# LukeFrankio/CiviWave-FEM

Hardware: AMD Instinct MI355X
Metric: PCG DOF-iterations/sec per Newmark step (PCG-it/s x DOFs); DOF-updates/s and K_eff HBM GB/s vs roofline reported alongside (higher is better)
Workload: dtype f32 SpMV, fp16-packed block-Jacobi, f64 reductions

## Files before the change

civiwave-fem_amd/csrc/cwf_internal.hpp:

```cpp
#pragma once

#include <hip/hip_runtime.h>

#include <cstdint>
#include <initializer_list>
#include <string>
#include <vector>

#include "../../include/cwf_hip.h"
#include "devmem.hpp"
#include "knobs.hpp"

namespace cwf
{

constexpr int kTileElems = 512;
constexpr int kMaxTileNodes = 512;
uint32_t hex_tile_lanes(uint64_t hexes);
#ifndef CWF_GROUP_SLOTS
#define CWF_GROUP_SLOTS 12
#endif
#ifndef CWF_GROUP_WAVES
#define CWF_GROUP_WAVES 1
#endif
// ... 195 lines not shown
    DevTiles t{};
};

struct Ctl
{
    double rho, alpha, beta, tol, res, rhs_norm, rhs_norm_raw, alpha_last, beta_last, denom, rr, rz;
    unsigned long long iterations;
    int active;
    int converged;
    int error;
    int error_iter;
    double rho2[2];
    double alpha_h[kXLag];
};

enum class PcgSchedule
{
    Parity,
    TwoKernel,
    Fused,
    FusedPeer,
    Resident,
};
struct SchedulePlan
{
    enum State
    {
        Unplanned,
        Local,
        Decided
    } state = Unplanned;
    unsigned grid = 0;
    int fused_knob = -1;
    PcgSchedule launch = PcgSchedule::TwoKernel;
    bool resident = false;
};

struct ResidentPlan
{
    unsigned G = 0, npt = 0, nph = 0;
    unsigned own_stride = 0, halo_stride = 0, npub = 0;
    size_t lds = 0;
    unsigned dims[3] = {0, 0, 0};
    unsigned max_own = 0, max_halo = 0;
    uint64_t halo_total = 0;
    const uint4 *hdr = nullptr, *own = nullptr, *halo = nullptr;
    const float4 *tcoef = nullptr;
    float *pub = nullptr;
    double *sh = nullptr;
    uint32_t tag = 1;
    bool shard = false;
    uint64_t remote_sends = 0;
    uint64_t ghost_total = 0;
};


const char *dashpot_update(const double C[9], double mass, double alpha, double dt, double P[9], double Q[9]);

}

struct cwf_hip_system
{
    cwf_hip_system() = default;
    cwf_hip_system(cwf_hip_system &&) = default;
    ~cwf_hip_system();
    int device = 0;
    hipStream_t stream = nullptr;
    int mode = CWF_MODE_PARITY;
    cwf::DevSys ds{};
    uint64_t reduction_block = 256;
    uint64_t reduction_partials = 1;
    cwf::DeviceArena mem;
    float *x = nullptr, *r = nullptr, *p = nullptr, *z = nullptr, *Ap = nullptr, *rhs = nullptr, *tmp = nullptr;
    float *p2 = nullptr, *p3 = nullptr, *p4 = nullptr;
    float *r2 = nullptr, *ap2 = nullptr;
    double *fsh = nullptr;
    double *g_fsh = nullptr;
    bool cls_global = false;
    bool unusable = false;
    int32_t px_send_k[2] = {-1, -1};
    uint32_t px_ebase = 0;
    cwf::SchedulePlan sched;
    cwf::ResidentPlan res;
    float *inv = nullptr;
    float *inv6 = nullptr;
    bool inv_fast = false;
    double inv_sK = 0.0, inv_sM = 0.0;
    double *part0 = nullptr, *part1 = nullptr, *part2 = nullptr;
    double *fgran = nullptr;
    uint32_t fgran_tag = 0;
    uint64_t part_cap = 0;
    uint32_t *perm = nullptr;
    float *pbuf = nullptr;
    cwf::Ctl *ctl = nullptr;
    cwf::Ctl *ctl_host = nullptr;
    double *scal = nullptr;
    cwf::DevicePtr<double> hist;
    uint64_t hist_cap = 0;
    uint64_t hist_count = 0;
    std::vector<uint32_t> lat_plane;
    uint64_t last_iters = 0, prev_iters = 0;
    std::string err, ctx;
    float *mo_blk = nullptr;
    uint32_t mo_cols = 0;
    double *mo_f64 = nullptr;
    float *mo_mass = nullptr;
// ... 228 lines not shown
```

civiwave-fem_amd/csrc/knobs.hpp:

```cpp
#pragma once

#include <cstdlib>
#include <cstring>

namespace cwf
{
struct Knob
{
    const char *name;
    const char *doc;
};

inline constexpr Knob kKnobs[] = {
    {"CWF_RENUMBER", "0: keep the caller's node order (no Morton / owner-tile renumbering)"},
    {"CWF_GEO", "0: the 48-B gradient records instead of recomputing geometry from tile-node coordinates"},
    {"CWF_GROUPS", "0: per-tet tiles (k_keff_tiles_pipe) instead of the fan groups"},
    {"CWF_GROUP_NT", "128: 128-lane fan-group tiles (default 256; tests/test_gpu_parity.py)"},
    {"CWF_TILE_ORDER", "morton|rcb: per-tet / hex8 tile order"},
    {"CWF_TILE_PIPE", "0: the one-tile-per-workgroup per-tet kernel (k_keff_tiles)"},
    {"CWF_HEX_NT", "128|256: lanes of the hex8 tiles (tests/test_hex8.py)"},
    {"CWF_LATTICE", "0: no structured-block stencil (lattice.cpp); structured Kuhn (hex8) blocks then run the fan groups (hex tiles)"},
    {"CWF_LAT_ZR", "0|1: the lattice update pass stores z / the K_eff pass forms z from r and the node class "
                   "(default: the latter from 2M nodes)"},
    {"CWF_LAT_L", "n: planes per lattice brick (default: about 1024 bricks of 256 threads, at least 4 planes)"},
    {"CWF_PARITY_TILES", "strip: PARITY node tiles of 256 consecutive nodes also on a single handle (default there: "
                         "compact breadth-first tiles and a separate p.Ap partials pass; shards always use strips)"},
    {"CWF_PARITY_STREAM", "0: the PARITY loop folds alpha / beta in their own kernels (k_pcg_alpha / k_pcg_beta) instead "
                          "of in workgroup 0 of the pass producing the chunk partials (kernels_parity.hip fold_stream)"},
    {"CWF_RESIDENT", "0: a structured block that fits on chip runs the launch-per-iteration schedules instead of the "
                     "resident one-launch solve (resident.hip; also off whenever CWF_FUSED is set)"},
    {"CWF_FUSED", "0: structured blocks run the two-kernel iteration (k_keff_lattice + k_pcg_update_tiles) instead of "
                  "the fused one-launch iteration (lattice_fused.inc); 2: fused also where the grid walks the work items "
                  "persistently (default: fused only where one round of workgroups covers them)"},
    {"CWF_PEER_FUSED", "0: a PEER shard's fused iteration exchanges through a k_peer_step launch after each fused launch "
                       "instead of inside the launch (lattice_fused.inc fused_peer_wait / fused_peer_publish)"},
    {"CWF_FUSED_TRACE", "path (ablation build only): per-workgroup phase stamps of one fused launch per solve, appended"},
    {"CWF_RESIDENT_TRACE", "path: per-workgroup phase stamps of one phase (CWF_FUSED_TRACE_IT) of every resident solve, "
                           "appended (tools/resident_trace.py)"},
    {"CWF_RESIDENT_REREAD", "1: every phase of the resident solve takes its first ring vote as failed once, so every ring "
                            "granule is requested and formed twice (tests/test_gpu_resident_handoff.py: same bits)"},
    {"CWF_FUSED_TRACE_IT", "n: the iteration whose launch CWF_FUSED_TRACE records (default 50)"},
    {"CWF_FUSED_MAXWG", "n: cap on the fused launch's grid (default 1024 workgroups; a grid below the work items walks them persistently)"},
    {"CWF_XLAG", "1..4: iterations per lazy x update (tests/test_gpu_parity.py compares 4 with 1)"},
    {"CWF_RCCL_LIB", "path: load this NCCL-API library instead of librccl (tests/transport: the host-staged "
                     "test transport that runs several ranks on one GPU, where RCCL refuses duplicate devices)"},
    {"CWF_TIMED_PCG", "bits: cwf_hip_keff_timed times the PCG-mode tiles kernel dry (tools/ablate.py)"},
    {"CWF_VERBOSE", "1: print the tiling statistics at create"},
};

inline const char *knob(const char *name)
{
    for (const Knob &k : kKnobs)
        if (std::strcmp(k.name, name) == 0)
            return std::getenv(name);
    return nullptr;
}
}
```

civiwave-fem_amd/csrc/lattice_common.hpp:

```cpp
#pragma once

#include <hip/hip_runtime.h>

#include <cstddef>
#include <type_traits>

#include "cwf_internal.hpp"
#include "keff_pick.hpp"
#include "reduce.hpp"

namespace cwf
{
namespace
{
typedef uint32_t u32x3 __attribute__((ext_vector_type(3)));
typedef float f2 __attribute__((ext_vector_type(2)));

__device__ __forceinline__ __amdgpu_buffer_rsrc_t ctl_rsrc(const Ctl *c)
{
    return __builtin_amdgcn_make_buffer_rsrc(const_cast<Ctl *>(c), 0, (int)sizeof(Ctl), 0x00020000);
}
__device__ __forceinline__ double ctl_f64(__amdgpu_buffer_rsrc_t rs, uint32_t off)
{
    const uint32_t lo = __builtin_amdgcn_raw_buffer_load_b32(rs, off, 0, 0),
// ... 28 lines not shown
struct LatHex
{
    static constexpr int nOff = kLatHexOffsets, nPairs = kLatHexPairs, coefPairs = 9 * kLatHexOffsets;
    static constexpr const int (&off)[kLatHexOffsets][3] = kLatHexOff;
    static constexpr int pair[kLatHexPairs][2] = {
#define P8(c) {c, 0}, {c, 1}, {c, 2}, {c, 3}, {c, 4}, {c, 5}, {c, 6}, {c, 7}
        P8(0), P8(1), P8(2), P8(3), P8(4), P8(5), P8(6), P8(7)
#undef P8
    };
    static constexpr const int (&pairOff)[kLatHexPairs] = kLatHexPairOff;
    static constexpr int pairStart[9] = {0, 8, 16, 24, 32, 40, 48, 56, 64};
};
template <bool HEX> using LatE = std::conditional_t<HEX, LatHex, LatKuhn>;
template <class E> constexpr const char *lat_kind() { return std::is_same_v<E, LatHex> ? "LatHex" : "LatKuhn"; }
constexpr uint32_t kLatOob3 = 0x15555555u;
constexpr uint32_t kLatOob1 = 0x3FFFFFFFu;

template <bool AFF>
__device__ __forceinline__ uint32_t lat_plane(const DevTiles &T, const uint32_t *__restrict__ plane, int k)
{
    if constexpr (AFF)
        return (uint32_t)k * T.lpstride;
    else
        return plane[k];
}

__device__ __forceinline__ __amdgpu_buffer_rsrc_t sized_rsrc(const void *base, uint32_t bytes)
{
    return __builtin_amdgcn_make_buffer_rsrc(const_cast<void *>(base), 0, (int)bytes, 0x00020000);
}

__device__ __forceinline__ void lat_z(const float4 A, const float2 B, uint32_t cls, const float r[3], float z[3])
{
    const float iv[9] = {A.x, A.y, A.z, A.y, A.w, B.x, A.z, B.x, B.y};
#pragma unroll
    for (int k = 0; k < 3; ++k)
    {
        const float zk = fmaf(iv[3 * k + 2], r[2], fmaf(iv[3 * k + 1], r[1], iv[3 * k] * r[0]));
        z[k] = (cls >> k) & 1u ? 0.0f : zk;
    }
}

enum
{
    kFR = 0,
    kFRR = 1,
    kFPA = 2,
    kFZA = 3,
    kFAMA = 4,
    kFusedShares = 5,
    kFusedSlot = 8
};

__device__ __forceinline__ bool fused_decide(Ctl *ctl, double *hist, unsigned j, const CtlPre &pre,
                                             const double v[kFusedShares], float *alpha_out, float *beta_out)
{
    const unsigned it = j - 1u;
    const double res = sqrt(v[kFRR]);
    const bool conv = it > 0 && res <= pre.tol;
    const double rho = v[kFR], denom = v[kFPA];
    const bool derr = !conv && fabs(denom) < 1.0e-18;
    const bool rerr = !conv && !derr && fabs(rho) < 1.0e-18;
    const double alpha = (conv || derr || rerr) ? 0.0 : rho / denom;
    const double rho_next = rho - 2.0 * alpha * v[kFZA] + alpha * alpha * v[kFAMA];
    const double beta = (conv || derr || rerr) ? 0.0 : rho_next / rho;
    if (blockIdx.x == 0 && threadIdx.x == 0)
    {
        if (it > 0)
        {
            ctl->res = res;
            ctl->iterations = it;
            hist[it] = res;
        }
        ctl->denom = denom;
        if (conv)
        {
            ctl->converged = 1;
            ctl->active = 0;
        }
        else if (derr)
        {
            ctl->error = CWF_ERR_DENOM_ZERO;
            ctl->error_iter = (int)it;
            ctl->active = 0;
        }
        else if (rerr)
        {
            ctl->error = CWF_ERR_RHO_ZERO;
            ctl->error_iter = (int)it;
            ctl->active = 0;
        }
        else
        {
            ctl->alpha = alpha;
            ctl->alpha_last = alpha;
            ctl->rho2[it & 1u] = rho;
            ctl->beta = beta;
            ctl->beta_last = beta;
        }
    }
    *alpha_out = (float)alpha;
    *beta_out = (float)beta;
    return !(conv || derr || rerr);
}

__device__ __forceinline__ void fused_form(const float4 *czA, const float2 *czB, uint32_t cls, float alpha,
                                           float beta, const float r[3], const float a[3], const float p[3],
                                           float rn[3], float z[3], float pn[3])
{
#pragma unroll
    for (int c = 0; c < 3; ++c)
        rn[c] = (cls >> c) & 1u ? 0.f : fmaf(-alpha, a[c], r[c]);
    lat_z(czA[cls], czB[cls], cls, rn, z);
#pragma unroll
    for (int c = 0; c < 3; ++c)
        pn[c] = fmaf(beta, p[c], z[c]);
}

__device__ __forceinline__ void fused_row_dots(const float4 *czA, const float2 *czB, uint32_t cls, const float u[3],
// ... 21 lines not shown
```

civiwave-fem_amd/csrc/lattice_fused.inc:

```

struct FusedArgs
{
    Ctl *ctl;
    const double *sin;
    unsigned nin;
    unsigned sin_stride, sis;
    double *sout;
    unsigned sstride;
    unsigned j;
    unsigned grid;
    double *hist;
    const float *rin;
    float *rout;
    const float *ain;
    float *aout;
    const float *pin;
    float *pout;
    float *x;
    unsigned px;
    FusedPeerArgs pe;
    uint64_t *trace;
};

constexpr uint64_t kFusedPeerTimeoutTicks = 10ull * 100000000ull;
// ... 54 lines not shown
    __shared__ int last_s;
    asm volatile("s_waitcnt vmcnt(0)" ::: "memory");
    __syncthreads();
    if (threadIdx.x == 0)
        last_s = __hip_atomic_fetch_add(pe.ticket, 1u, __ATOMIC_RELAXED, __HIP_MEMORY_SCOPE_AGENT) + 1u == gridDim.x;
    __syncthreads();
    if (!last_s)
        return;
    __builtin_amdgcn_fence(__ATOMIC_ACQUIRE, "");
    double v[kFusedShares];
    fold_k<NT, kFusedShares>(fa.sout, gridDim.x, fa.sstride, red, v);
    if (threadIdx.x < kFusedSlot)
    {
        double t = 0.0;
#pragma unroll
        for (int q = 0; q < kFusedShares; ++q)
            t = threadIdx.x == (unsigned)q ? v[q] : t;
        for (uint32_t p = 0; p < pe.nranks; ++p)
            __hip_atomic_store(pe.gdst[p] + threadIdx.x, t, __ATOMIC_RELAXED, __HIP_MEMORY_SCOPE_SYSTEM);
    }
    asm volatile("s_waitcnt vmcnt(0)" ::: "memory");
    __syncthreads();
    if (threadIdx.x == 0)
    {
        __builtin_amdgcn_fence(__ATOMIC_RELEASE, "");
        for (uint32_t p = 0; p < pe.nranks; ++p)
            if (p != pe.rank)
                __hip_atomic_store(pe.flag[p], pe.epoch, __ATOMIC_RELAXED, __HIP_MEMORY_SCOPE_SYSTEM);
        __hip_atomic_store(pe.done, pe.epoch, __ATOMIC_RELAXED, __HIP_MEMORY_SCOPE_SYSTEM);
        __hip_atomic_store(pe.ticket, 0u, __ATOMIC_RELAXED, __HIP_MEMORY_SCOPE_AGENT);
    }
}

__device__ __forceinline__ void st3_sys(__amdgpu_buffer_rsrc_t rs, uint32_t byteoff, const float v[3])
{
    const u32x3 w = {__float_as_uint(v[0]), __float_as_uint(v[1]), __float_as_uint(v[2])};
    __builtin_amdgcn_raw_buffer_store_b96(w, rs, byteoff, 0, 17);
}

template <int NT>
__device__ __forceinline__ bool fused_scalars(const FusedArgs &fa, const CtlPre &pre, double *red, float *alpha_out,
                                              float *beta_out)
{
    if (fa.j == 0)
    {
        *alpha_out = 0.f;
        *beta_out = 0.f;
        return pre.active != 0;
    }
    double v[kFusedShares];
    fold_k<NT, kFusedShares>(fa.sin, fa.nin, fa.sin_stride, red, v, fa.sis);
    if (!pre.active)
        return false;
    return fused_decide(fa.ctl, fa.hist, fa.j, pre, v, alpha_out, beta_out);
}

struct FusedFill
{
    float r[2][3], a[2][3], p[2][3];
    uint32_t c[2];
    float x[3], m;
};

struct FusedKeep
{
    float z[3], m;
    uint32_t c;
};

template <class E, bool AFF, bool SHARD>
__device__ __forceinline__ void fused_shell_node(const DevSys &s, const FusedArgs &fa, const float *__restrict__ coef,
                                                 const uint32_t *__restrict__ plane, uint32_t q, float alpha,
                                                 float beta, const float4 *czA, const float2 *czB,
                                                 double d[kFusedShares])
{
    const DevTiles &T = s.t;
    const int nx = (int)T.lnx, ny = (int)T.lny, nz = (int)T.lnz;
    int i, j, k;
    uint32_t rq = q;
    const uint32_t full = (uint32_t)(nx * ny), per = (uint32_t)(2 * nx + 2 * (ny - 2));
    const uint32_t nlo = T.lk0 == 0 ? full : 0u, nmid = (T.lkI1 - T.lkI0) * per;
    if (rq < nlo)
    {
        k = 0;
        i = (int)(rq % (uint32_t)nx);
        j = (int)(rq / (uint32_t)nx);
    }
    else if ((rq -= nlo) < nmid)
    {
        k = (int)(T.lkI0 + rq / per);
        rq %= per;
        if (rq < (uint32_t)nx)
            i = (int)rq, j = 0;
        else if (rq < 2u * nx)
            i = (int)rq - nx, j = ny - 1;
        else if (rq < 2u * nx + (uint32_t)(ny - 2))
            i = 0, j = 1 + (int)rq - 2 * nx;
        else
            i = nx - 1, j = 1 + (int)rq - 2 * nx - (ny - 2);
    }
    else
    {
        rq -= nmid;
        k = nz - 1;
        i = (int)(rq % (uint32_t)nx);
        j = (int)(rq / (uint32_t)nx);
    }
// ... 577 lines not shown
```

civiwave-fem_amd/csrc/resident.cpp:

```cpp
#include <algorithm>
#include <cstdio>
#include <cstring>

#include "abi_internal.hpp"

namespace cwf
{
namespace
{
constexpr unsigned kResThreads = 512, kResOwn = 4 * kResThreads, kResHalo = 3 * kResThreads;
constexpr unsigned kResTypesHost = 12;
constexpr unsigned kResGhostHost = 512;
constexpr uint32_t kNone = 0xFFFFFFFFu;
constexpr uint32_t kResGhost = 0x80000000u;
constexpr unsigned kFusedSharesHost = 5;

void split(unsigned n, unsigned g, unsigned q, unsigned &a, unsigned &b)
{
    a = (unsigned)((uint64_t)n * q / g);
    b = (unsigned)((uint64_t)n * (q + 1) / g);
}
}

bool plan_resident(cwf_hip_system *h, bool shard)
// ... 160 lines not shown
                    for (int o = 1; o < noff; ++o)
                    {
                        const long ii = (long)i + off[o][0], jj = (long)j + off[o][1], kk = (long)k + off[o][2];
                        if (!inside(ii, jj, kk))
                            continue;
                        const uint32_t m = node((unsigned)ii, (unsigned)jj, (unsigned)kk);
                        if (owner[m] == b || seen[m] == b)
                            continue;
                        seen[m] = b;
                        const unsigned slot = (unsigned)((kk - (long)q[4] + 1) * PXY + (jj - (long)q[2] + 1) * PX +
                                                         (ii - (long)q[0] + 1));
                        const uint32_t src = m >= Nown ? kResGhost | (m - Nown) : pubidx[m];
                        halol[b].push_back(uint4{m, slot, src, 0u});
                    }
        std::sort(halol[b].begin(), halol[b].end(), [](const uint4 &a, const uint4 &c) { return a.z < c.z; });
        max_halo = std::max<unsigned>(max_halo, (unsigned)halol[b].size());
        halo_total += halol[b].size();
        const auto g0 = std::find_if(halol[b].begin(), halol[b].end(), [](const uint4 &e) { return (e.z & kResGhost) != 0; });
        const uint64_t ng = (uint64_t)(halol[b].end() - g0);
        if (ng > kResGhostHost)
            return false;
        hdr[b].y = (uint32_t)(g0 - halol[b].begin());
        ghost_total += ng;
    }
    const bool small0 = (max_own + kResThreads - 1) / kResThreads <= 3 && (max_halo + kResThreads - 1) / kResThreads <= 2;
    std::vector<uint8_t> btypes((size_t)G * kResTypesHost, 0);
    for (unsigned b = 0; b < G && !small0; ++b)
    {
        int idx[27];
        std::fill(idx, idx + 27, -1);
        unsigned nt = 0;
        for (const uint4 &e : ownl[b])
            idx[cls[e.x] >> 3] = 0;
        for (unsigned ty = 0; ty < 27; ++ty)
            if (idx[ty] == 0 && ty != 13)
            {
                if (nt == kResTypesHost)
                    return false;
                btypes[(size_t)b * kResTypesHost + nt] = (uint8_t)ty;
                idx[ty] = (int)nt++;
            }
        for (uint4 &e : ownl[b])
        {
            const unsigned ty = cls[e.x] >> 3;
            e.y |= (ty == 13 ? 0u : (uint32_t)idx[ty]) << 24;
        }
    }
    const unsigned npt = (max_own + kResThreads - 1) / kResThreads, nph = (max_halo + kResThreads - 1) / kResThreads;
    if (max_own > kResOwn || max_halo > kResHalo || max_slots > slot_cap(max_own, max_halo) || N - Nown >= kResGhost)
        return false;
    const bool small = npt <= 3 && nph <= 2;
    const unsigned own_stride = (small ? 3u : 4u) * kResThreads, halo_stride = (small ? 2u : 3u) * kResThreads;
    const size_t lds = max_slots * 16;
    if (resident_blocks_per_cu(h->ds, npt, nph, lds, shard) < 1)
        return false;
    std::vector<uint4> own((size_t)G * own_stride, uint4{kNone, 0u, kNone, kNone}),
        halo((size_t)G * halo_stride, uint4{kNone, 0u, kNone, 0u});
    for (unsigned b = 0; b < G; ++b)
    {
        std::copy(ownl[b].begin(), ownl[b].end(), own.begin() + (size_t)b * own_stride);
        std::copy(halol[b].begin(), halol[b].end(), halo.begin() + (size_t)b * halo_stride);
    }
    const int npairs = t.lhex ? kLatHexPairs : kLatPairs;
    std::vector<float> cf((size_t)(noff + npairs) * 9);
    if (hipMemcpy(cf.data(), t.lcoef, cf.size() * sizeof(float), hipMemcpyDeviceToHost) != hipSuccess)
        return false;
    std::vector<float4> tco(27ull * noff * 3, float4{0.f, 0.f, 0.f, 0.f});
    for (unsigned ty = 0; ty < 27; ++ty)
    {
        const unsigned sd[3] = {ty % 3, (ty / 3) % 3, ty / 9};
        unsigned w8 = 0;
        for (unsigned c8 = 0; c8 < 8; ++c8)
        {
            bool in = true;
            for (int ax = 0; ax < 3; ++ax)
                in = in && (((c8 >> ax) & 1u) ? sd[ax] != 0 : sd[ax] != 2);
            w8 |= (in ? 1u : 0u) << c8;
        }
        for (int o = 1; o < noff; ++o)
        {
            double S[9] = {};
            for (int pp = 0; pp < npairs; ++pp)
            {
                const int c = t.lhex ? pp / 8 : kLatPair[pp][0];
                const int po = t.lhex ? kLatHexPairOff[pp] : kLatPairOff[pp];
                if (po != o || !((w8 >> c) & 1u))
                    continue;
                for (int e = 0; e < 9; ++e)
                    S[e] += (double)cf[(size_t)9 * noff + 9 * pp + e];
            }
            float4 *q = &tco[(size_t)3 * (ty * noff + o)];
            q[0] = float4{(float)S[0], (float)S[3], (float)S[1], (float)S[4]};
            q[1] = float4{(float)S[2], (float)S[5], (float)S[6], (float)S[7]};
            q[2] = float4{(float)S[8], 0.f, 0.f, 0.f};
        }
    }
    std::vector<float4> btco(small ? 0 : (size_t)G * kResTypesHost * noff * 3, float4{0.f, 0.f, 0.f, 0.f});
    for (unsigned b = 0; b < G && !small; ++b)
        for (unsigned k = 0; k < kResTypesHost; ++k)
            std::copy(tco.begin() + (size_t)3 * noff * btypes[(size_t)b * kResTypesHost + k],
                      tco.begin() + (size_t)3 * noff * (btypes[(size_t)b * kResTypesHost + k] + 1),
                      btco.begin() + ((size_t)b * kResTypesHost + k) * 3 * noff);
    float4 *dtc;
    if (small ? upload(h, &dtc, tco.data(), tco.size()) : upload(h, &dtc, btco.data(), btco.size()))
        return false;
    uint4 *dh, *dow, *dha;
    float *dpub;
    double *dsh;
    if (upload(h, &dh, hdr.data(), hdr.size()) || upload(h, &dow, own.data(), own.size()) ||
        upload(h, &dha, halo.data(), halo.size()) || dalloc(h, &dpub, 2ull * 12 * std::max<uint32_t>(npub, 1u)) ||
        dalloc(h, &dsh, 2ull * 2 * kFusedSharesHost * G))
        return false;
    if (hipMemset(dsh, 0, 2ull * 2 * kFusedSharesHost * G * sizeof(double)) != hipSuccess ||
        hipMemset(dpub, 0, 2ull * 12 * std::max<uint32_t>(npub, 1u) * sizeof(float)) != hipSuccess)
        return false;
    if (shard && peer_resident_clear(h))
        return false;
    rp.G = G;
    rp.npt = small ? 3 : 4;
    rp.nph = small ? 2 : 3;
    rp.own_stride = own_stride;
    rp.halo_stride = halo_stride;
    rp.npub = std::max<uint32_t>(npub, 1u);
    rp.lds = lds;
    std::memcpy(rp.dims, bg, sizeof bg);
    rp.max_own = max_own;
    rp.max_halo = max_halo;
    rp.halo_total = halo_total;
    rp.hdr = dh;
    rp.tcoef = dtc;
    rp.own = dow;
    rp.halo = dha;
    rp.pub = dpub;
    rp.sh = dsh;
    rp.shard = shard;
    rp.remote_sends = remote_sends;
    rp.ghost_total = ghost_total;
    if (knob("CWF_VERBOSE"))
        fprintf(stderr, "[cwf] resident plan: %u boxes (%u x %u x %u), max_own %u, max_halo %u, %u published nodes\n", G,
                bg[0], bg[1], bg[2], max_own, max_halo, npub);
    return true;
}

uint64_t resident_offchip_bytes(const cwf_hip_system *h)
{
    const ResidentPlan &rp = h->res;
    uint64_t b = 48ull * (rp.halo_total - rp.ghost_total + rp.npub) + 16ull * (rp.ghost_total + rp.remote_sends) +
                 80ull * rp.G * (1ull + rp.G);
    if (rp.shard)
        b += 80ull * h->nranks * (1ull + rp.G);
    return b;
}

}
```

civiwave-fem_amd/csrc/resident.hip:

```cpp
#include <hip/hip_ext.h>

#include <cstdio>
#include <cstdlib>
#include <vector>

#include "lattice_common.hpp"

namespace cwf
{
namespace
{
constexpr int kResNT = 512;
constexpr uint32_t kResMaxRounds = 4000000u;
constexpr uint32_t kResNone = 0xFFFFFFFFu;
constexpr uint32_t kResOob = 0xFFFFFF00u;
constexpr uint32_t kResGhost = 0x80000000u;
constexpr int kResTypes = 12;
typedef uint32_t u32x4 __attribute__((ext_vector_type(4)));

struct ResArgs
{
    Ctl *ctl;
    double *hist;
    const uint4 *hdr;
    const uint4 *own;
    const uint4 *halo;
    const float4 *tcoef;
    uint32_t own_stride, halo_stride;
    float *pub;
    uint32_t npub;
    double *sh;
    uint32_t tag0;
    float *x, *r;
    uint32_t max_it;
    uint64_t *trace;
    uint32_t trace_j;
    uint32_t reread;
    ResPeerArgs pa;
};

__device__ __forceinline__ void st4_sc1(__amdgpu_buffer_rsrc_t rs, uint32_t off, u32x4 w)
{
    __builtin_amdgcn_raw_buffer_store_b128(w, rs, off, 0, 16);
}
__device__ __forceinline__ u32x4 pk4(float a, float b, float c, float d)
{
    return u32x4{__float_as_uint(a), __float_as_uint(b), __float_as_uint(c), __float_as_uint(d)};
}
__device__ __forceinline__ u32x4 ld4_sc1(__amdgpu_buffer_rsrc_t rs, uint32_t off)
{
    return __builtin_amdgcn_raw_buffer_load_b128(rs, off, 0, 16);
}
__device__ __forceinline__ void st4_sys(__amdgpu_buffer_rsrc_t rs, uint32_t off, u32x4 w)
{
    __builtin_amdgcn_raw_buffer_store_b128(w, rs, off, 0, 17);
}
__device__ __forceinline__ u32x4 ld4_sys(__amdgpu_buffer_rsrc_t rs, uint32_t off)
{
    return __builtin_amdgcn_raw_buffer_load_b128(rs, off, 0, 17);
}

__device__ __forceinline__ void lds_sync()
{
    __builtin_amdgcn_fence(__ATOMIC_RELEASE, "workgroup", "local");
    __builtin_amdgcn_s_barrier();
    __builtin_amdgcn_fence(__ATOMIC_ACQUIRE, "workgroup", "local");
}

template <int NT, int K>
__device__ __forceinline__ void block_sum_lds(double v[K], double *red)
{
#pragma unroll
    for (int q = 0; q < K; ++q)
    {
        v[q] = wave_sum(v[q]);
        if ((threadIdx.x & 63) == 0)
            red[K * (threadIdx.x >> 6) + q] = v[q];
    }
    lds_sync();
#pragma unroll
    for (int q = 0; q < K; ++q)
    {
        double t = 0.0;
#pragma unroll
        for (int w = 0; w < NT / 64; ++w)
            t += red[K * w + q];
        v[q] = t;
    }
}

template <bool SYM, class E, int NPT, int NPH, bool MR>
__global__ __launch_bounds__(kResNT) __attribute__((amdgpu_waves_per_eu(2, 2))) void k_pcg_resident(DevSys s, ResArgs ra, const float *__restrict__ coef)
{
    extern __shared__ float4 pl[];
    __shared__ double red[kFusedShares * (kResNT / 64)];
    __shared__ float4 czA[kLatClasses];
    __shared__ float2 czB[kLatClasses];
    constexpr bool LST = NPT > 3;
    constexpr int kTT = LST ? kResTypes : 27;
    __shared__ float4 tcf[kTT * E::nOff * 3];
    __shared__ int vote[3];
    __shared__ double rt[MR ? kFusedShares * kMaxPeers : 1];
    __shared__ float st[LST ? 9 : 1][LST ? NPT * kResNT : 1];
    float sreg[LST ? 1 : NPT][LST ? 1 : 12];
    const auto S = [&](int u, int q) -> float & {
        if constexpr (LST)
            return st[q][threadIdx.x + (uint32_t)u * kResNT];
        else
            return sreg[u][q];
    };
    const DevTiles &T = s.t;
    const uint32_t G = gridDim.x, b = blockIdx.x, tid = threadIdx.x;
    const uint4 hd = ra.hdr[b];
    const int PX = (int)hd.z, PXY = (int)hd.w;
    const auto stamp = [&](unsigned j, int i) {
        if (ra.trace && j == ra.trace_j && tid == 0)
            __hip_atomic_store(ra.trace + 8ull * b + i, __builtin_amdgcn_s_memrealtime(), __ATOMIC_RELAXED,
                               __HIP_MEMORY_SCOPE_AGENT);
    };
    for (uint32_t i = tid; i < hd.x; i += kResNT)
        pl[i] = float4{0.f, 0.f, 0.f, 0.f};
    for (uint32_t i = tid; i < (uint32_t)(kTT * E::nOff * 3); i += kResNT)
        tcf[i] = ra.tcoef[(LST ? (size_t)b * (kTT * E::nOff * 3) : 0) + i];

    if (tid < kLatClasses)
    {
        const float4 zA = T.lcz[2u * tid], zB = T.lcz[2u * tid + 1u];
        czA[tid] = zA;
        czB[tid] = float2{zB.x, zB.y};
    }
    const uint32_t vbytes = 12u * s.N;
    constexpr bool multi = MR;
    const __amdgpu_buffer_rsrc_t rx = sized_rsrc(ra.x, vbytes), rr = sized_rsrc(ra.r, vbytes),
                                 rcls = sized_rsrc(T.lcls, s.N), rmass = sized_rsrc(s.mass, 4u * s.N),
                                 rpub = sized_rsrc(ra.pub, 32u * ra.npub), rsh = sized_rsrc(ra.sh, 160u * G);
    uint32_t on[NPT], osc[NPT], opub[NPT];
    float m[NPT];
#pragma unroll
    for (int u = 0; u < NPT; ++u)
    {
        const uint32_t e0 = tid + (uint32_t)u * kResNT;
        const uint4 e = ra.own[(size_t)b * ra.own_stride + e0];
        on[u] = e.x;
        opub[u] = e.z;
        const bool v = e.x != kResNone;
        const uint32_t nb = v ? 12u * e.x : 12u * kLatOob3;
        const u32x3 wr = __builtin_amdgcn_raw_buffer_load_b96(rr, nb, 0, 0),
                    wx = __builtin_amdgcn_raw_buffer_load_b96(rx, nb, 0, 0);
        S(u, 0) = __uint_as_float(wr.x), S(u, 1) = __uint_as_float(wr.y), S(u, 2) = __uint_as_float(wr.z);
        S(u, 3) = S(u, 4) = S(u, 5) = 0.f;
        S(u, 6) = __uint_as_float(wx.x), S(u, 7) = __uint_as_float(wx.y), S(u, 8) = __uint_as_float(wx.z);
        if constexpr (!LST)
            sreg[u][9] = sreg[u][10] = sreg[u][11] = 0.f;
        osc[u] = (e.y & (LST ? 0xFF00FFFFu : 0xFFFFu)) |
                 (uint32_t)__builtin_amdgcn_raw_buffer_load_b8(rcls, v ? e.x : kResNone, 0, 0) << 16;
        m[u] = __uint_as_float(__builtin_amdgcn_raw_buffer_load_b32(rmass, v ? 4u * e.x : 4u * kLatOob1, 0, 0));
    }
    uint32_t hn[NPH], hsc[NPH], hpub[NPH];
    float hr[NPH][3], hp[NPH][3];
#pragma unroll
    for (int h = 0; h < NPH; ++h)
    {
        const uint4 e = ra.halo[(size_t)b * ra.halo_stride + tid + (uint32_t)h * kResNT];
        hn[h] = e.x;
        hpub[h] = e.z;
        hsc[h] = e.y | (uint32_t)__builtin_amdgcn_raw_buffer_load_b8(rcls, e.x != kResNone ? e.x : kResNone, 0, 0)
                           << 16;
#pragma unroll
        for (int c = 0; c < 3; ++c)
            hr[h][c] = hp[h][c] = 0.f;
    }
    const CtlPre pre = ctl_prefetch(ra.ctl, 1u);
    int soff[E::nOff];
#pragma unroll
    for (int o = 0; o < E::nOff; ++o)
        soff[o] = E::off[o][0] + E::off[o][1] * PX + E::off[o][2] * PXY;
    const auto request = [&](int h, uint32_t par, u32x4 &c) {
        const bool gh = (hpub[h] & kResGhost) != 0u, v = hn[h] != kResNone;
        c = ld4_sc1(rpub, v && !gh ? 16u * (par * ra.npub + hpub[h]) : kResOob);
        if constexpr (multi)
        {
            const __amdgpu_buffer_rsrc_t rg = sized_rsrc(par ? ra.pa.grecv[1] : ra.pa.grecv[0], ra.pa.grecv_bytes);
            c |= ld4_sys(rg, v && gh ? 16u * (hpub[h] & ~kResGhost) : kResOob);
        }
    };
    __syncthreads();
    const float sK = (float)s.sK, sM = (float)s.sM;
    bool go = pre.active != 0;
    unsigned j = 0;
    for (; go; ++j)
    {
        float alpha = 0.f, beta = 0.f;
        float ha[NPH][3], hrn[NPH][3], hpn[NPH][3];
        u32x4 w1[NPH];
        const uint32_t par = (j - 1u) & 1u, want = ra.tag0 + j;
        uint32_t round = 0;
        const auto all_ok = [&](bool ok) {
            if (tid == 0)
                vote[(round + 1u) % 3u] = 1;
            if (!ok)
                vote[round % 3u] = 0;
            lds_sync();
            return vote[round % 3u] != 0;
        };
        const auto give_up = [&]() {
            if (tid == 0)
            {
                ra.ctl->error = CWF_ERR_HIP;
                ra.ctl->error_iter = (int)j;
                ra.ctl->active = 0;
            }
        };
        if (j == 0)
        {
#pragma unroll
            for (int h = 0; h < NPH; ++h)
            {
                const u32x3 w = __builtin_amdgcn_raw_buffer_load_b96(rr, hn[h] != kResNone ? 12u * hn[h] : 12u * kLatOob3,
                                                                     0, 0);
                hr[h][0] = __uint_as_float(w.x), hr[h][1] = __uint_as_float(w.y), hr[h][2] = __uint_as_float(w.z);
#pragma unroll
                for (int c = 0; c < 3; ++c)
                    ha[h][c] = 0.f;
            }
        }
        else
        {
            stamp(j, 0);
            u32x4 g[kFusedShares];
            for (;; ++round)
            {
#pragma unroll
                for (int q = 0; q < kFusedShares; ++q)
                    g[q] = ld4_sc1(rsh, tid < G ? 16u * ((par * G + tid) * kFusedShares + (uint32_t)q) : kResOob);
                bool ok = true;
#pragma unroll
                for (int q = 0; q < kFusedShares; ++q)
                    ok = ok && (tid >= G || g[q].z == want);
                if (all_ok(ok))
                    break;
                if (round >= kResMaxRounds)
                {
                    give_up();
                    return;
                }
                __builtin_amdgcn_s_sleep(2);
            }
#pragma unroll
            for (int h = 0; h < NPH; ++h)
                request(h, par, w1[h]);
            stamp(j, 1);
            double v[kFusedShares];
#pragma unroll
            for (int q = 0; q < kFusedShares; ++q)
                v[q] = tid < G ? __hiloint2double((int)g[q].y, (int)g[q].x) : 0.0;
            block_sum_lds<kResNT, kFusedShares>(v, red);
            if constexpr (multi)
            {
                const uint32_t nr = ra.pa.nranks, jp = j & 1u;
                if (b == 0 && tid < (uint32_t)kFusedShares)
                {
                    double t = v[0];
#pragma unroll
                    for (int q = 1; q < kFusedShares; ++q)
                        t = tid == (uint32_t)q ? v[q] : t;
                    const u32x4 w = {(uint32_t)__double2loint(t), (uint32_t)__double2hiint(t), want, 0u};
#pragma unroll
                    for (int p = 0; p < kMaxPeers; ++p)
                        if ((uint32_t)p < nr)
                            st4_sys(sized_rsrc(jp ? ra.pa.tot[p][1] : ra.pa.tot[p][0], 80u * nr),
                                    16u * (kFusedShares * ra.pa.rank + tid), w);
                }
                const __amdgpu_buffer_rsrc_t rtm = sized_rsrc(jp ? ra.pa.tot_mine[1] : ra.pa.tot_mine[0], 80u * nr);
                u32x4 gt;
                for (;; ++round)
                {
                    gt = ld4_sys(rtm, tid < kFusedShares * nr ? 16u * tid : kResOob);
                    if (all_ok(tid >= kFusedShares * nr || gt.z == want))
                        break;
                    if (round >= kResMaxRounds)
                    {
                        give_up();
                        return;
                    }
                    __builtin_amdgcn_s_sleep(2);
                }
                if (tid < kFusedShares * nr)
                    rt[tid] = __hiloint2double((int)gt.y, (int)gt.x);
                lds_sync();
#pragma unroll
                for (int q = 0; q < kFusedShares; ++q)
                {
                    double t = 0.0;
                    for (uint32_t p = 0; p < nr; ++p)
                        t += rt[kFusedShares * p + q];
                    v[q] = t;
                }
            }
            stamp(j, 7);
            go = fused_decide(ra.ctl, ra.hist, j, pre, v, &alpha, &beta);
            if (go && j - 1u == ra.max_it)
                go = false;
            if (!go)
                break;
            stamp(j, 2);
        }
#pragma unroll
        for (int u = 0; u < NPT; ++u)
            asm volatile("" : "+v"(osc[u]), "+v"(opub[u]), "+v"(on[u]));
#pragma unroll
        for (int h = 0; h < NPH; ++h)
            asm volatile("" : "+v"(hsc[h]), "+v"(hpub[h]), "+v"(hn[h]));
        double d[kFusedShares] = {0.0, 0.0, 0.0, 0.0, 0.0};
#pragma unroll
        for (int u = 0; u < NPT; ++u)
        {
            __builtin_amdgcn_sched_barrier(0);
            if (on[u] == kResNone)
                continue;
            const uint32_t slot = osc[u] & 0xFFFFu;
            const float4 po = LST ? pl[slot] : float4{S(u, 9), S(u, 10), S(u, 11), 0.f};
            const float rr0[3] = {S(u, 0), S(u, 1), S(u, 2)}, aa0[3] = {S(u, 3), S(u, 4), S(u, 5)},
                        pp0[3] = {po.x, po.y, po.z};
            float rn[3], zz[3], pn[3];
            fused_form(czA, czB, LST ? (osc[u] >> 16) & 0xFFu : osc[u] >> 16, alpha, beta, rr0, aa0, pp0, rn, zz, pn);
#pragma unroll
            for (int c = 0; c < 3; ++c)
            {
                S(u, 6 + c) = fmaf(alpha, pp0[c], S(u, 6 + c));
                S(u, c) = rn[c];
                if constexpr (!LST)
                    S(u, 9 + c) = pn[c];
            }
            pl[slot] = float4{pn[0], pn[1], pn[2], 0.f};
            fused_entry_dots(rn, zz, d);
        }
        bool again = ra.reread != 0u && j > 0;
        for (;; ++round)
        {
            bool hok = true;
#pragma unroll
            for (int h = 0; h < NPH; ++h)
            {
                if (hn[h] == kResNone)
                    continue;
                if (j > 0)
                {
                    if (w1[h].w != want)
                    {
                        hok = false;
                        continue;
                    }
                    ha[h][0] = __uint_as_float(w1[h].x), ha[h][1] = __uint_as_float(w1[h].y);
// ... 149 lines not shown
        const u32x3 vx = {__float_as_uint(S(u, 6)), __float_as_uint(S(u, 7)), __float_as_uint(S(u, 8))},
                    vr = {__float_as_uint(S(u, 0)), __float_as_uint(S(u, 1)), __float_as_uint(S(u, 2))};
        __builtin_amdgcn_raw_buffer_store_b96(vx, wx, nb, 0, 0);
        __builtin_amdgcn_raw_buffer_store_b96(vr, wr, nb, 0, 0);
    }
}

using ResidentFn = void (*)(DevSys, ResArgs, const float *);

template <bool SYM, class E, int NPT, int NPH, bool MR> Pick<ResidentFn> resident_pick()
{
    static const std::string name = kernel_name("k_pcg_resident", SYM, lat_kind<E>(), NPT, NPH, MR);
    return {k_pcg_resident<SYM, E, NPT, NPH, MR>, name.c_str()};
}

Pick<ResidentFn> pick_resident(const DevSys &s, bool small, bool shard)
{
    return with_bools(
        [](auto sm, auto mr, auto hex, auto sym) {
            return resident_pick<sym(), LatE<hex()>, sm() ? 3 : 4, sm() ? 2 : 3, mr()>();
        },
        small, shard, s.t.lhex != 0, s.t.lsym != 0);
}
inline bool resident_small(unsigned npt, unsigned nph) { return npt <= 3 && nph <= 2; }
}

size_t resident_static_lds(const DevSys &s, bool small, bool shard)
{
    hipFuncAttributes a{};
    const void *k = reinterpret_cast<const void *>(pick_resident(s, small, shard).fn);
    return hipFuncGetAttributes(&a, k) == hipSuccess ? a.sharedSizeBytes : 0;
}

int resident_blocks_per_cu(const DevSys &s, unsigned npt, unsigned nph, size_t lds, bool shard)
{
    if (npt > 4 || nph > 3)
        return 0;
    int bpc = 0;
    const ResidentFn k = pick_resident(s, resident_small(npt, nph), shard).fn;
    if (hipFuncSetAttribute(reinterpret_cast<const void *>(k), hipFuncAttributeMaxDynamicSharedMemorySize, (int)lds) !=
            hipSuccess ||
        hipOccupancyMaxActiveBlocksPerMultiprocessor(&bpc, k, kResNT, lds) != hipSuccess)
        return 0;
    return bpc;
}

const char *resident_kernel_name(const DevSys &s, const ResidentPlan &rp)
{
    return pick_resident(s, resident_small(rp.npt, rp.nph), rp.shard).name;
}

void launch_pcg_resident(cwf_hip_system *h, uint32_t max_it, hipStream_t st, hipEvent_t e0, hipEvent_t e1)
{
    const ResidentPlan &rp = h->res;
    ResArgs ra{};
    ra.ctl = h->ctl;
    ra.hist = h->hist;
    ra.hdr = rp.hdr;
    ra.own = rp.own;
    ra.halo = rp.halo;
    ra.tcoef = rp.tcoef;
    ra.own_stride = rp.own_stride;
    ra.halo_stride = rp.halo_stride;
    ra.pub = rp.pub;
    ra.npub = rp.npub;
    ra.sh = rp.sh;
    ra.tag0 = h->res.tag;
    ra.x = h->x;
    ra.r = h->r;
    ra.max_it = max_it;
    if (rp.shard)
        peer_resident_args(h, ra.pa);
    else
        ra.pa = ResPeerArgs{};
    static uint64_t *trace = nullptr;
    static unsigned trace_n = 0;
    const char *tp = knob("CWF_RESIDENT_TRACE");
    if (tp && trace_n < rp.G)
    {
        if (trace)
            (void)hipFree(trace);
        trace = nullptr;
        trace_n = hipMalloc(reinterpret_cast<void **>(&trace), 64ull * rp.G) == hipSuccess ? rp.G : 0u;
    }
    if (tp && trace)
    {
        const char *at = knob("CWF_FUSED_TRACE_IT");
        ra.trace = trace;
        ra.trace_j = at ? (uint32_t)atoi(at) : 50u;
        (void)hipMemsetAsync(trace, 0, 64ull * rp.G, st);
    }
    const char *rk = knob("CWF_RESIDENT_REREAD");
    ra.reread = rk && rk[0] == '1' ? 1u : 0u;
    launch_kernel(pick_resident(h->ds, resident_small(rp.npt, rp.nph), rp.shard).fn, rp.G, kResNT, rp.lds, st, e0, e1,
                  h->ds, ra, h->ds.t.lcoef);
    if (tp && trace)
    {
        std::vector<uint64_t> v(8ull * rp.G);
        if (hipStreamSynchronize(st) == hipSuccess &&
            hipMemcpy(v.data(), trace, v.size() * sizeof(uint64_t), hipMemcpyDeviceToHost) == hipSuccess)
            if (FILE *f = std::fopen(tp, "a"))
            {
                std::fprintf(f, "# resident phase %u grid %u boxes %ux%ux%u\n", ra.trace_j, rp.G, rp.dims[0], rp.dims[1],
                             rp.dims[2]);
                for (unsigned b = 0; b < rp.G; ++b)
                {
                    std::fprintf(f, "%u", b);
                    for (int i = 0; i < 8; ++i)
                        std::fprintf(f, " %llu", (unsigned long long)v[8ull * b + i]);
                    std::fprintf(f, "\n");
                }
                std::fclose(f);
            }
    }
}

}
```

Measured before the change: 99.14 billion.

## Offload resident PCG share fold and decision to a dedicated reducer workgroup

Adds an extra workgroup to the resident one-launch PCG solve. It polls the per-box partial shares, folds them, runs the alpha/beta convergence decision once, and publishes the result in a small decision slot inside the publish buffer. The worker boxes no longer each gather and fold all G boxes' shares. They poll only their halo data and the decision slot, which is meant to cut redundant reduction traffic and latency on the critical path. It is enabled by default for unsharded plans with at least 56 boxes and spare co-resident capacity. The cost is an extra hop through global memory for the decision, one more workgroup that must be co-resident, and the trace buffer moving into plan-owned storage.

```diff
diff --git a/civiwave-fem_amd/csrc/cwf_internal.hpp b/civiwave-fem_amd/csrc/cwf_internal.hpp
--- a/civiwave-fem_amd/csrc/cwf_internal.hpp
+++ b/civiwave-fem_amd/csrc/cwf_internal.hpp
@@ -271,6 +271,10 @@
     bool shard = false;
     uint64_t remote_sends = 0;
     uint64_t ghost_total = 0;
+    unsigned capacity = 0;
+    uint32_t dec_off = 0;
+    DevicePtr<uint64_t> trace;
+    unsigned trace_n = 0;
 };
 
 
diff --git a/civiwave-fem_amd/csrc/knobs.hpp b/civiwave-fem_amd/csrc/knobs.hpp
--- a/civiwave-fem_amd/csrc/knobs.hpp
+++ b/civiwave-fem_amd/csrc/knobs.hpp
@@ -39,7 +39,10 @@
                            "appended (tools/resident_trace.py)"},
     {"CWF_RESIDENT_REREAD", "1: every phase of the resident solve takes its first ring vote as failed once, so every ring "
                             "granule is requested and formed twice (tests/test_gpu_resident_handoff.py: same bits)"},
-    {"CWF_FUSED_TRACE_IT", "n: the iteration whose launch CWF_FUSED_TRACE records (default 50)"},
+    {"CWF_RESIDENT_REDUCER", "0|1, read at every launch: the resident solve's share fold and decision by one extra workgroup on a "
+                             "spare CU, never / wherever the plan is eligible (unsharded, >= 2 boxes, one more workgroup "
+                             "co-resident); default: eligible and at least kResReducerMinBoxes boxes (resident.hip)"},
+    {"CWF_FUSED_TRACE_IT","n: the iteration whose launch CWF_FUSED_TRACE records (default 50)"},
     {"CWF_FUSED_MAXWG", "n: cap on the fused launch's grid (default 1024 workgroups; a grid below the work items walks them persistently)"},
     {"CWF_XLAG", "1..4: iterations per lazy x update (tests/test_gpu_parity.py compares 4 with 1)"},
     {"CWF_RCCL_LIB", "path: load this NCCL-API library instead of librccl (tests/transport: the host-staged "
diff --git a/civiwave-fem_amd/csrc/lattice_common.hpp b/civiwave-fem_amd/csrc/lattice_common.hpp
--- a/civiwave-fem_amd/csrc/lattice_common.hpp
+++ b/civiwave-fem_amd/csrc/lattice_common.hpp
@@ -104,7 +104,7 @@
     kFusedSlot = 8
 };
 
-__device__ __forceinline__ bool fused_decide(Ctl *ctl, double *hist, unsigned j, const CtlPre &pre,
+__device__ __forceinline__ bool fused_decide(Ctl *ctl, double *hist, unsigned j, const CtlPre &pre, bool writer,
                                              const double v[kFusedShares], float *alpha_out, float *beta_out)
 {
     const unsigned it = j - 1u;
@@ -116,7 +116,7 @@
     const double alpha = (conv || derr || rerr) ? 0.0 : rho / denom;
     const double rho_next = rho - 2.0 * alpha * v[kFZA] + alpha * alpha * v[kFAMA];
     const double beta = (conv || derr || rerr) ? 0.0 : rho_next / rho;
-    if (blockIdx.x == 0 && threadIdx.x == 0)
+    if (writer)
     {
         if (it > 0)
         {
diff --git a/civiwave-fem_amd/csrc/lattice_fused.inc b/civiwave-fem_amd/csrc/lattice_fused.inc
--- a/civiwave-fem_amd/csrc/lattice_fused.inc
+++ b/civiwave-fem_amd/csrc/lattice_fused.inc
@@ -130,7 +130,7 @@
     fold_k<NT, kFusedShares>(fa.sin, fa.nin, fa.sin_stride, red, v, fa.sis);
     if (!pre.active)
         return false;
-    return fused_decide(fa.ctl, fa.hist, fa.j, pre, v, alpha_out, beta_out);
+    return fused_decide(fa.ctl, fa.hist, fa.j, pre, blockIdx.x == 0 && threadIdx.x == 0, v, alpha_out, beta_out);
 }
 
 struct FusedFill
diff --git a/civiwave-fem_amd/csrc/resident.cpp b/civiwave-fem_amd/csrc/resident.cpp
--- a/civiwave-fem_amd/csrc/resident.cpp
+++ b/civiwave-fem_amd/csrc/resident.cpp
@@ -236,7 +236,8 @@
     const bool small = npt <= 3 && nph <= 2;
     const unsigned own_stride = (small ? 3u : 4u) * kResThreads, halo_stride = (small ? 2u : 3u) * kResThreads;
     const size_t lds = max_slots * 16;
-    if (resident_blocks_per_cu(h->ds, npt, nph, lds, shard) < 1)
+    const int bpc = resident_blocks_per_cu(h->ds, npt, nph, lds, shard);
+    if (bpc < 1)
         return false;
     std::vector<uint4> own((size_t)G * own_stride, uint4{kNone, 0u, kNone, kNone}),
         halo((size_t)G * halo_stride, uint4{kNone, 0u, kNone, 0u});
@@ -320,6 +321,9 @@
     rp.shard = shard;
     rp.remote_sends = remote_sends;
     rp.ghost_total = ghost_total;
+    rp.capacity = (unsigned)bpc * G0;
+    const uint64_t dec = (32ull * rp.npub + 127u) / 128u * 128u;
+    rp.dec_off = dec + 256u <= 96ull * rp.npub && dec + 256u < 0xFFFFFF00ull ? (uint32_t)dec : 0u;
     if (knob("CWF_VERBOSE"))
         fprintf(stderr, "[cwf] resident plan: %u boxes (%u x %u x %u), max_own %u, max_halo %u, %u published nodes\n", G,
                 bg[0], bg[1], bg[2], max_own, max_halo, npub);
diff --git a/civiwave-fem_amd/csrc/resident.hip b/civiwave-fem_amd/csrc/resident.hip
--- a/civiwave-fem_amd/csrc/resident.hip
+++ b/civiwave-fem_amd/csrc/resident.hip
@@ -15,6 +15,7 @@
 constexpr uint32_t kResNone = 0xFFFFFFFFu;
 constexpr uint32_t kResOob = 0xFFFFFF00u;
 constexpr uint32_t kResGhost = 0x80000000u;
+constexpr unsigned kResReducerMinBoxes = 56;
 constexpr int kResTypes = 12;
 typedef uint32_t u32x4 __attribute__((ext_vector_type(4)));
 
@@ -36,6 +37,9 @@
     uint64_t *trace;
     uint32_t trace_j;
     uint32_t reread;
+    uint32_t G;
+    uint32_t reducer;
+    uint32_t dec_off;
     ResPeerArgs pa;
 };
 
@@ -86,6 +90,101 @@
         for (int w = 0; w < NT / 64; ++w)
             t += red[K * w + q];
         v[q] = t;
+    }
+}
+
+constexpr uint32_t kDecGo = 1u, kDecStop = 2u, kDecFailed = 3u;
+
+__device__ __forceinline__ void resident_reduce(const ResArgs &ra, double *red2, int *flag)
+{
+    const uint32_t G = ra.G, tid = threadIdx.x;
+    const __amdgpu_buffer_rsrc_t rsh = sized_rsrc(ra.sh, 160u * G),
+                                 rdec = sized_rsrc(reinterpret_cast<const char *>(ra.pub) + ra.dec_off, 256u);
+    const CtlPre pre = ctl_prefetch(ra.ctl, 1u);
+    const bool tr = ra.trace != nullptr;
+    if (tid == 0)
+        flag[1] = 0;
+    lds_sync();
+    if (pre.active == 0)
+        return;
+    for (unsigned j = 1;; ++j)
+    {
+        const uint32_t par = (j - 1u) & 1u, want = ra.tag0 + j;
+        const bool st = tr && j == ra.trace_j;
+        uint64_t t0 = 0;
+        if (st)
+            t0 = __builtin_amdgcn_s_memrealtime();
+        if (tid == 0)
+            flag[(j + 1u) % 3u] = 0;
+        u32x4 g[kFusedShares];
+        uint32_t rounds = 0;
+        for (;; ++rounds)
+        {
+#pragma unroll
+            for (int q = 0; q < kFusedShares; ++q)
+                g[q] = ld4_sc1(rsh, tid < G ? 16u * ((par * G + tid) * kFusedShares + (uint32_t)q) : kResOob);
+            bool ok = true;
+#pragma unroll
+            for (int q = 0; q < kFusedShares; ++q)
+                ok = ok && (tid >= G || g[q].z == want);
+            if (__builtin_amdgcn_ballot_w64(!ok) == 0ull)
+                break;
+            if (rounds >= kResMaxRounds)
+            {
+                flag[j % 3u] = 1;
+                break;
+            }
+            __builtin_amdgcn_s_sleep(1);
+        }
+        double *red = red2 + (j & 1u) * (kFusedShares * (kResNT / 64));
+        if (st && (tid & 63u) == 0u)
+            reinterpret_cast<uint64_t *>(red2 + 2 * kFusedShares * (kResNT / 64))[tid >> 6] = __builtin_amdgcn_s_memrealtime();
+        double v[kFusedShares];
+#pragma unroll
+        for (int q = 0; q < kFusedShares; ++q)
+            v[q] = tid < G ? __hiloint2double((int)g[q].y, (int)g[q].x) : 0.0;
+        block_sum_lds<kResNT, kFusedShares>(v, red);
+        const bool failed = flag[j % 3u] != 0;
+        uint64_t t2 = 0;
+        if (st)
+            t2 = __builtin_amdgcn_s_memrealtime();
+        float alpha = 0.f, beta = 0.f;
+        bool go = false;
+        if (failed)
+        {
+            if (tid == 0)
+            {
+                ra.ctl->error = CWF_ERR_HIP;
+                ra.ctl->error_iter = (int)j;
+                ra.ctl->active = 0;
+            }
+        }
+        else
+        {
+            go = fused_decide(ra.ctl, ra.hist, j, pre, tid == 0, v, &alpha, &beta);
+            if (go && j - 1u == ra.max_it)
+                go = false;
+        }
+        if (tid == 64u)
+            st4_sc1(rdec, 128u * (j & 1u),
+                    u32x4{__float_as_uint(alpha), __float_as_uint(beta), failed ? kDecFailed : go ? kDecGo : kDecStop, want});
+        if (st && tid == 64u)
+            __hip_atomic_store(ra.trace + 8ull * G + 3, __builtin_amdgcn_s_memrealtime(), __ATOMIC_RELAXED,
+                               __HIP_MEMORY_SCOPE_AGENT);
+        if (st && tid == 0)
+        {
+            const uint64_t *ws = reinterpret_cast<const uint64_t *>(red2 + 2 * kFusedShares * (kResNT / 64));
+            uint64_t t1 = 0;
+            for (int w = 0; w < kResNT / 64; ++w)
+                t1 = ws[w] > t1 ? ws[w] : t1;
+            uint64_t *row = ra.trace + 8ull * G;
+            __hip_atomic_store(row + 0, t0, __ATOMIC_RELAXED, __HIP_MEMORY_SCOPE_AGENT);
+            __hip_atomic_store(row + 1, t1, __ATOMIC_RELAXED, __HIP_MEMORY_SCOPE_AGENT);
+            __hip_atomic_store(row + 2, t2, __ATOMIC_RELAXED, __HIP_MEMORY_SCOPE_AGENT);
+            __hip_atomic_store(row + 4, __builtin_amdgcn_s_memrealtime(), __ATOMIC_RELAXED, __HIP_MEMORY_SCOPE_AGENT);
+        }
+        if (!go)
+            return;
     }
 }
 
@@ -110,7 +209,13 @@
             return sreg[u][q];
     };
     const DevTiles &T = s.t;
-    const uint32_t G = gridDim.x, b = blockIdx.x, tid = threadIdx.x;
+    const uint32_t G = ra.G, b = blockIdx.x, tid = threadIdx.x;
+    if constexpr (!MR)
+        if (ra.reducer != 0u && b == G)
+        {
+            resident_reduce(ra, reinterpret_cast<double *>(tcf), vote);
+            return;
+        }
     const uint4 hd = ra.hdr[b];
     const int PX = (int)hd.z, PXY = (int)hd.w;
     const auto stamp = [&](unsigned j, int i) {
@@ -175,8 +280,8 @@
 #pragma unroll
     for (int o = 0; o < E::nOff; ++o)
         soff[o] = E::off[o][0] + E::off[o][1] * PX + E::off[o][2] * PXY;
-    const auto request = [&](int h, uint32_t par, u32x4 &c) {
-        const bool gh = (hpub[h] & kResGhost) != 0u, v = hn[h] != kResNone;
+    const auto request = [&](int h, uint32_t par, u32x4 &c, bool need = true) {
+        const bool gh = (hpub[h] & kResGhost) != 0u, v = need && hn[h] != kResNone;
         c = ld4_sc1(rpub, v && !gh ? 16u * (par * ra.npub + hpub[h]) : kResOob);
         if constexpr (multi)
         {
@@ -224,6 +329,48 @@
                     ha[h][c] = 0.f;
             }
         }
+        else if (!MR && ra.reducer != 0u)
+        {
+            stamp(j, 0);
+            const __amdgpu_buffer_rsrc_t rdec = sized_rsrc(reinterpret_cast<const char *>(ra.pub) + ra.dec_off, 256u);
+            u32x4 dg;
+#pragma unroll
+            for (int h = 0; h < NPH; ++h)
+                w1[h] = u32x4{0u, 0u, 0u, ~want};
+            for (;; ++round)
+            {
+#pragma unroll
+                for (int h = 0; h < NPH; ++h)
+                {
+                    const bool need = w1[h].w != want;
+                    u32x4 c;
+                    request(h, par, c, need);
+                    w1[h] = need ? c : w1[h];
+                }
+                dg = ld4_sc1(rdec, 128u * (j & 1u));
+                if (all_ok(dg.w == want))
+                    break;
+                if (round >= kResMaxRounds)
+                {
+                    give_up();
+                    return;
+                }
+                __builtin_amdgcn_s_sleep(2);
+            }
+            stamp(j, 1);
+            stamp(j, 7);
+            stamp(j, 2);
+            const uint32_t state = __builtin_amdgcn_readfirstlane(dg.z);
+            if (state == kDecFailed)
+                return;
+            alpha = __uint_as_float(__builtin_amdgcn_readfirstlane(dg.x));
+            beta = __uint_as_float(__builtin_amdgcn_readfirstlane(dg.y));
+            if (state != kDecGo)
+            {
+                go = false;
+                break;
+            }
+        }
         else
         {
             stamp(j, 0);
@@ -298,7 +445,7 @@
                 }
             }
             stamp(j, 7);
-            go = fused_decide(ra.ctl, ra.hist, j, pre, v, &alpha, &beta);
+            go = fused_decide(ra.ctl, ra.hist, j, pre, b == 0 && tid == 0, v, &alpha, &beta);
             if (go && j - 1u == ra.max_it)
                 go = false;
             if (!go)
@@ -554,7 +701,7 @@
 
 void launch_pcg_resident(cwf_hip_system *h, uint32_t max_it, hipStream_t st, hipEvent_t e0, hipEvent_t e1)
 {
-    const ResidentPlan &rp = h->res;
+    ResidentPlan &rp = h->res;
     ResArgs ra{};
     ra.ctl = h->ctl;
     ra.hist = h->hist;
@@ -575,37 +722,37 @@
         peer_resident_args(h, ra.pa);
     else
         ra.pa = ResPeerArgs{};
-    static uint64_t *trace = nullptr;
-    static unsigned trace_n = 0;
+    const bool eligible = !rp.shard && rp.G >= 2u && rp.G + 1u <= rp.capacity && rp.dec_off != 0u;
+    const char *rdk = knob("CWF_RESIDENT_REDUCER");
+    ra.G = rp.G;
+    ra.reducer = eligible && (rdk ? rdk[0] == '1' : rp.G >= kResReducerMinBoxes) ? 1u : 0u;
+    ra.dec_off = rp.dec_off;
+    const unsigned grid = rp.G + ra.reducer;
     const char *tp = knob("CWF_RESIDENT_TRACE");
-    if (tp && trace_n < rp.G)
-    {
-        if (trace)
-            (void)hipFree(trace);
-        trace = nullptr;
-        trace_n = hipMalloc(reinterpret_cast<void **>(&trace), 64ull * rp.G) == hipSuccess ? rp.G : 0u;
-    }
-    if (tp && trace)
+    if (tp && rp.trace_n < grid)
+        rp.trace_n = rp.trace.alloc(8ull * grid) == hipSuccess ? grid : 0u;
+    uint64_t *trace = tp && rp.trace_n >= grid ? rp.trace.get() : nullptr;
+    if (trace)
     {
         const char *at = knob("CWF_FUSED_TRACE_IT");
         ra.trace = trace;
         ra.trace_j = at ? (uint32_t)atoi(at) : 50u;
-        (void)hipMemsetAsync(trace, 0, 64ull * rp.G, st);
+        (void)hipMemsetAsync(trace, 0, 64ull * grid, st);
     }
     const char *rk = knob("CWF_RESIDENT_REREAD");
     ra.reread = rk && rk[0] == '1' ? 1u : 0u;
-    launch_kernel(pick_resident(h->ds, resident_small(rp.npt, rp.nph), rp.shard).fn, rp.G, kResNT, rp.lds, st, e0, e1,
+    launch_kernel(pick_resident(h->ds, resident_small(rp.npt, rp.nph), rp.shard).fn, grid, kResNT, rp.lds, st, e0, e1,
                   h->ds, ra, h->ds.t.lcoef);
-    if (tp && trace)
-    {
-        std::vector<uint64_t> v(8ull * rp.G);
+    if (trace)
+    {
+        std::vector<uint64_t> v(8ull * grid);
         if (hipStreamSynchronize(st) == hipSuccess &&
             hipMemcpy(v.data(), trace, v.size() * sizeof(uint64_t), hipMemcpyDeviceToHost) == hipSuccess)
             if (FILE *f = std::fopen(tp, "a"))
             {
-                std::fprintf(f, "# resident phase %u grid %u boxes %ux%ux%u\n", ra.trace_j, rp.G, rp.dims[0], rp.dims[1],
-                             rp.dims[2]);
-                for (unsigned b = 0; b < rp.G; ++b)
+                std::fprintf(f, "# resident phase %u grid %u reducer %u boxes %ux%ux%u\n", ra.trace_j, grid, ra.reducer,
+                             rp.dims[0], rp.dims[1], rp.dims[2]);
+                for (unsigned b = 0; b < grid; ++b)
                 {
                     std::fprintf(f, "%u", b);
                     for (int i = 0; i < 8; ++i)
```

Result: faster. 107.1 billion (median of 6 runs) (+8.0%).
